# keillernogueira/dynamic-rs-segmentation

Measured on AMD Instinct MI355X. Metric: training patches/sec dilated_grsl_rate8 64x64x5, higher is better.
Workload: dtype f32; 1 GPU; dilated_grsl_rate8 (Dilated8Pooling) training step, single_fixed 64x64, 5-band synthetic 2048x2048 tile, global batch 128 (crop+augment+normalise, fwd, loss, bwd, momentum, confusion); global_batch=128, patch=64, bands=5, classes=6, parallelism=dp1, sync_bn=True, rccl_ranks_observed=1

## Files before the change

dynamic-rs-segmentation_amd/_lib.py:

```python
import ctypes as C
import os

_HERE = os.path.dirname(os.path.abspath(__file__))
LIB_PATH = os.path.join(_HERE, "libdrs_hip.so")
DEV_LIB_PATH = os.path.join(_HERE, "libdrs_hip_dev.so")

_p, _i, _f, _d = C.c_void_p, C.c_int, C.c_float, C.c_double
_sz, _u64 = C.c_size_t, C.c_ulonglong

SIGNATURES = {
    "drs_conv_mtile": (_i, [_i]),
    "drs_conv_forward": (_i, [_p, _i, _i, _i, _i, _i, _p, _p, _i, _i, _i, _i, _i, _p, _i, _i, _i, _p, _p]),
    "drs_conv_workspace_floats": (_sz, [_i]),
    "drs_conv_halo_skip": (_i, [_i, _i, _i, _i, _i, _i, _i]),
    "drs_conv_executed_ksteps": (_i, [_i, _i, _i, _i, _i, _i, _i, _p, _p]),
    "drs_conv_forward_ws": (_i, [_p, _i, _i, _i, _i, _i, _p, _p, _i, _i, _i, _i, _i, _p, _i, _i, _i, _p, _p, _sz, _p]),
    "drs_conv_wgrad_splits": (_i, [_i, _i, _i, _i, _i]),
    "drs_conv_wgrad": (_i, [_p, _i, _i, _i, _i, _i, _p, _i, _i, _i, _i, _i, _i, _i, _i, _i, _p, _p, _p]),
    "drs_filter_flip_transpose": (_i, [_p, _p, _i, _i, _i, _p]),
    "drs_filter_pad_cin": (_i, [_p, _p, _i, _i, _i, _i, _p]),
    "drs_split_conv_mtile": (_i, [_i]),
    "drs_split_terms": (_i, [_p, _sz, _i, _p, _p]),
    "drs_filter_split": (_i, [_p, _i, _i, _i, _i, _i, _p, _p, _p]),
    "drs_conv_forward_split": (_i, [_p, _i, _i, _i, _i, _i, _p, _p, _i, _i, _i, _i, _i, _p, _i, _i, _i, _p, _i, _p]),
# ... 74 lines not shown
    "drs_polygon_rings": (_i, [_p, _p, _i, _i, _i, _i, _p, _p, _p]),
    "drs_polygon_write": (_i, [_p, _i, _i, _i, _i, _i, _p, _p, _p, _p]),
    "drs_distance_scratch_bytes": (_sz, [_i, _i]),
    "drs_distance_transform": (_i, [_p, _p, _i, _i, _i, _i, _i, _p, _p, _sz, _p]),
    "drs_surface_scratch_bytes": (_sz, [_i, _i]),
    "drs_surface_histogram": (_i, [_p, _p, _i, _i, _i, _i, _p, _p, _sz, _p]),
    "drs_patch_boundary_weight": (_i, [_p, _p, _i, _i, _i, _d, _d, _p, _p, _p]),
    "drs_classifier_loss_pixel": (_i, [_p, _i, _i, _i, _i, _i, _i, _i, _p, _p, _p, _p, _p, _f, _p, _f, _p, _p, _p, _p, _i, _i, _p, _p,
                                       _p, _p, _p]),
    "drs_patch_dice_coeffs": (_i, [_p, _p, _p, _i, _i, _i, _d, _d, _d, _d, _p, _p, _p, _p]),
    "drs_classifier_loss_dice": (_i, [_p, _i, _i, _i, _i, _i, _i, _i, _p, _p, _p, _p, _p, _f, _p, _f, _p, _p, _p, _p, _p, _i, _i, _p,
                                      _p, _p, _p, _p]),
    "drs_dice_loss_add": (_i, [_p, _i, _p, _p]),
    "drs_patch_hard_weight": (_i, [_p, _p, _p, _p, _i, _i, _i, _d, _i, _p, _p, _p, _p]),
    "drs_lovasz_scratch_bytes": (_sz, [_i, _i, _i]),
    "drs_patch_lovasz_grad": (_i, [_p, _p, _p, _p, _i, _i, _i, _d, _p, _p, _p, _p, _p, _sz, _p]),
    "drs_classifier_loss_region": (_i, [_p, _i, _i, _i, _i, _i, _i, _i, _p, _p, _p, _p, _p, _f, _p, _f, _p, _p, _p, _p, _p, _i, _i, _p,
                                        _p, _p, _p, _p]),
    "drs_surface_loss_scratch_bytes": (_sz, [_i, _i, _i]),
    "drs_patch_surface_loss": (_i, [_p, _p, _p, _p, _i, _i, _i, _d, _d, _p, _i, _p, _p, _p, _p, _sz, _p]),
    "drs_net_create": (_i, [C.c_char_p, _i, _i, _f, _i, _i, _i, _f, C.POINTER(_p)]),
    "drs_net_destroy": (None, [_p]),
    "drs_net_num_buffers": (_i, [_p]),
    "drs_net_buffer_info": (_i, [_p, _i, C.c_char_p, _i, C.POINTER(_sz), C.POINTER(_i)]),
    "drs_net_bind": (_i, [_p, C.c_char_p, _p, _sz]),
    "drs_net_buffer": (_i, [_p, C.c_char_p, C.POINTER(_p), C.POINTER(_sz)]),
    "drs_net_layout": (_i, [_p, C.POINTER(_sz), C.POINTER(_sz), C.POINTER(_sz), C.POINTER(_i), C.POINTER(_i), C.POINTER(_i)]),
    "drs_net_layer_info": (_i, [_p, _i, C.c_char_p, _i, C.POINTER(_i), C.c_char_p, C.c_char_p, _i, C.POINTER(_i), C.POINTER(_i)]),
    "drs_net_info": (_i, [_p, C.c_char_p, _i, C.POINTER(_f), C.POINTER(_i), C.c_char_p, _i, C.POINTER(_i), C.POINTER(_i)]),
    "drs_net_receptive_field": (_i, [_p, C.POINTER(_i), C.POINTER(_i)]),
    "drs_net_receptive_field_gated": (_i, [_p, C.POINTER(_i), C.POINTER(_i)]),
    "drs_net_se_info": (_i, [_p, _i, C.c_char_p, _i, C.POINTER(_i), C.POINTER(_i), C.POINTER(_i)]),
    "drs_net_type_name": (_i, [_i, C.c_char_p, _i, C.POINTER(_i)]),
    "drs_net_num_variables": (_i, [_p]),
    "drs_net_variable_info": (_i, [_p, _i, C.c_char_p, _i, C.POINTER(_sz), C.POINTER(_sz), C.POINTER(_i), C.POINTER(_i)]),
    "drs_params_get": (_i, [_p, C.c_char_p, C.c_char_p, _p, _sz, _p]),
    "drs_params_set": (_i, [_p, C.c_char_p, C.c_char_p, _p, _sz, _p]),
    "drs_grad_buffer": (_i, [_p, C.POINTER(_p), C.POINTER(_sz)]),
    "drs_net_global_step": (C.c_longlong, [_p, C.c_longlong]),
    "drs_net_learning_rate": (_f, [_p, _f]),
    "drs_net_set_comm": (_i, [_p, _i, _i, _p, _p, _p]),
    "drs_rccl_bind_library": (_i, [C.c_char_p]),
    "drs_rccl_available": (_i, []),
    "drs_rccl_form": (_i, []),
    "drs_rccl_unique_id": (_i, [_p]),
    "drs_rccl_comm_create": (_i, [_i, _i, _p, C.POINTER(_p)]),
    "drs_rccl_comm_destroy": (_i, [_p]),
    "drs_rccl_all_reduce": (_i, [_p, _p, C.c_size_t, _i, _p]),
    "drs_net_set_rccl": (_i, [_p, _i, _i, _p, _p, _p]),
    "drs_train_step": (_i, [_p, _i, _i, _f, _i, _d, _p]),
    "drs_forward": (_i, [_p, _i, _i, _i, _i, _p]),
    "drs_apply_update": (_i, [_p, _f, _p]),
    "drs_forward_staged": (_i, [_p, _i, _i, _i, _p, _i, _i, _p]),
    "drs_net_se_gate_finish": (_i, [_p, _i, _d, _p]),
    "drs_net_set_two_streams": (_i, [_p, _i]),
    "drs_net_set_class_weights": (_i, [_p, _p, _i]),
    "drs_net_get_class_weights": (_i, [_p, _p, _i, C.POINTER(_i)]),
    "drs_net_set_focal_gamma": (_i, [_p, _f]),
    "drs_net_get_focal_gamma": (_i, [_p, C.POINTER(_f)]),
    "drs_net_set_boundary_weight": (_i, [_p, _d, _d, _i]),
    "drs_net_get_boundary_weight": (_i, [_p, C.POINTER(_d), C.POINTER(_d), C.POINTER(_i)]),
    "drs_net_set_dice": (_i, [_p, _d, _d, _d, _d]),
    "drs_net_get_dice": (_i, [_p, C.POINTER(_d), C.POINTER(_d), C.POINTER(_d), C.POINTER(_d)]),
    "drs_net_set_hard_mining": (_i, [_p, _d, _i]),
    "drs_net_get_hard_mining": (_i, [_p, C.POINTER(_d), C.POINTER(_i)]),
    "drs_net_set_lovasz": (_i, [_p, _d]),
    "drs_net_get_lovasz": (_i, [_p, C.POINTER(_d)]),
    "drs_net_set_surface_loss": (_i, [_p, _d, _d]),
    "drs_net_get_surface_loss": (_i, [_p, C.POINTER(_d), C.POINTER(_d)]),
    "drs_net_timing": (_i, [_p, _i]),
    "drs_net_num_timing_kinds": (_i, []),
    "drs_net_timing_summary": (_i, [_p, _i, C.c_char_p, _i, C.POINTER(_i), C.POINTER(_d), C.POINTER(_d)]),
}
ALLREDUCE_FN = C.CFUNCTYPE(_i, _p, _p, _sz, _i, _i, _p)
WAIT_FN = C.CFUNCTYPE(_i, _p, _i, _p)
WANT_LOGITS, WITH_LABELS, USE_ACC_MASK, USE_LOSS_MASK, NO_UPDATE = 1, 2, 4, 8, 16


DEV_SIGNATURES = {
    "drs_debug_skip_taps": (_i, [_i]), "drs_debug_conv_variant": (_i, [_i]), "drs_debug_conv_wide192": (_i, [_i]),
    "drs_debug_conv_splitk": (_i, [_i]), "drs_debug_conv_hybrid": (_i, [_i]), "drs_debug_conv_sk_order": (_i, [_i]), "drs_debug_conv_prio": (_i, [_i]),
    "drs_debug_conv_sk_geometry": (_i, [_i, _i, _i, _p]), "drs_debug_conv_trace": (_i, [_p]), "drs_debug_conv_lpt": (_i, [_i]), "drs_debug_conv_order": (_i, [_i] * 7 + [_p, _i]),
    "drs_debug_conv_image_tiles": (_i, [_i]), "drs_debug_conv_order_image": (_i, [_i] * 7 + [_p, _i]),
    "drs_debug_wgrad_variant": (_i, [_i]), "drs_debug_wgrad_seg": (_i, [_i]), "drs_debug_wgrad_balance": (_i, [_i]), "drs_debug_wgrad_target": (_i, [_i]),
    "drs_debug_wgrad_len": (_i, [_i]), "drs_debug_wgrad_minchunks": (_i, [_i]), "drs_debug_wgrad_prio": (_i, [_i]), "drs_debug_cls_variant": (_i, [_i]), "drs_debug_slide_blocks": (_i, [_i]), "drs_debug_slide_minrows": (_i, [_i]), "drs_debug_slide_rowpad": (_i, [_i]), "drs_debug_chain_mode": (_i, [_i]), "drs_debug_jitter": (_i, [C.c_ulonglong]), "drs_debug_wg_stream_prio": (_i, [_i]), "drs_debug_reductions_on_chain": (_i, [_i]), "drs_debug_wgrad_schedule": (_i, [_i, _i, _i]), "drs_debug_variant": (_i, [_i]),
    "drs_debug_wgrad_cut": (_i, [_i] * 7 + [_p, _i, _p, _p]),
}


class DrsError(RuntimeError):
    pass


_lib = None
_dev = None


def _open(path, signatures):
    if not os.path.isfile(path):
        raise DrsError("HIP library not built: %s is missing (run dynamic-rs-segmentation_amd/csrc/build.sh "
                       "or __graft_entry__.build()); there is no CPU fallback" % path)
    import torch
    lib = C.CDLL(path)
    for name, (res, args) in signatures.items():
        fn = getattr(lib, name)
        fn.restype = res
        fn.argtypes = args
    return lib


def load():
    global _lib
    if _lib is None:
        _lib = _open(LIB_PATH, SIGNATURES)
    return _lib


class _Dev(object):

    def __init__(self, lib):
        self.lib = lib

    def __getattr__(self, name):
        return getattr(self.lib, name)

    def load(self):
        return self.lib

    def call(self, name, *args):
        rc = getattr(self.lib, name)(*args)
        if rc != 0:
            raise DrsError("%s -> %s" % (name, _STATUS.get(rc, rc)))

    def query(self, name, *args):
        return getattr(self.lib, name)(*args)


def dev():
    global _dev
    if _dev is None:
        sig = dict(SIGNATURES)
        sig.update(DEV_SIGNATURES)
        _dev = _Dev(_open(DEV_LIB_PATH, sig))
    return _dev


_STATUS = {1: "DRS_ERR_ARG (rejected argument)", 2: "DRS_ERR_HIP (launch failed)"}


def call(name, *args):
    rc = getattr(load(), name)(*args)
    if rc != 0:
        raise DrsError("%s -> %s" % (name, _STATUS.get(rc, rc)))


def query(name, *args):
    return getattr(load(), name)(*args)
```

dynamic-rs-segmentation_amd/csrc/conv_mfma.hip:

```cpp
#include "drs_common.hpp"
#include <algorithm>
#include <cstdlib>
#include <map>
#include <mutex>
#include <numeric>
#include <tuple>
#include <vector>

namespace {

constexpr int BK = 32;
constexpr int LDA = BK + 4;

struct ConvArgs {
  const float* in; int S, P, ld_in, coff_in;
  int M;
  const float* w;
  const float* bias;
  float* out; int ld_out, coff_out;
  float* stats;
  int k, rate, pad, Cin, Cout;
  int accumulate;
  int skip_halo;
  float rcpS, rcpSS;
  float* sk_slab;
  int sk_W, sk_nks, sk_U;
  int sk_T, sk_tiles, sk_G, sk_order;
  int prio;
  int lpt_T, lpt_ta, lpt_tb, lpt_P;
  int img_g;
  const int* img_order;
#ifdef DRS_DEV
  unsigned long long* trace;
#endif
};

__device__ __forceinline__ void set_prio_by_progress(int done, int total, int& quarter, int mode = 1) {
  const int q = __builtin_amdgcn_readfirstlane((done * 4) / total);
  if (q == quarter) return;
  quarter = q;
  if (mode == 2) {
    if (q <= 0) __builtin_amdgcn_s_setprio(2);
    else if (q == 1) __builtin_amdgcn_s_setprio(1);
    else __builtin_amdgcn_s_setprio(0);
    return;
  }
  if (q <= 0) __builtin_amdgcn_s_setprio(3);
  else if (q == 1) __builtin_amdgcn_s_setprio(2);
  else if (q == 2) __builtin_amdgcn_s_setprio(1);
  else __builtin_amdgcn_s_setprio(0);
}

__host__ __device__ __forceinline__ int lpt_tile(int wg, int T, int ta, int tb, int P, int ntn) {
  const int per = P * T * ntn, nI = tb - ta, nE = T - nI;
  const int chunk = wg / per;
  int wl = wg - chunk * per, p, t;
  if (wl < P * nI * ntn) {
    p = wl / (nI * ntn);
    wl -= p * nI * ntn;
    t = ta + wl / ntn;
  } else {
    wl -= P * nI * ntn;
    p = wl / (nE * ntn);
    wl -= p * nE * ntn;
    const int e = wl / ntn;
    t = e < ta ? e : tb + (e - ta);
  }
  return ((chunk * P + p) * T + t) * ntn + wl % ntn;
}

__host__ __device__ __forceinline__ int sk_first_unit(int w, int U, int W) { return (int)((long long)w * U / W); }
__host__ __device__ __forceinline__ int sk_owner(int x, int U, int W) { return (int)((((long long)x + 1) * W - 1) / U); }

template <int BM, int BN, int WM, int WN, bool MAP = false>
__device__ __forceinline__ void conv_epilogue(const ConvArgs& a, f32x16 (&acc)[BM / WM / 32][BN / WN / 32], float* scratch, int m0, int n0,
                                              int pix0 = 0, int pcs = 30) {
  constexpr int WTM = BM / WM, WTN = BN / WN;
  constexpr int TM = WTM / 32, TN = WTN / 32;
  const int t = threadIdx.x;
  const int lane = t & 63, wave = t >> 6;
  const int li = lane & 31, h = lane >> 5;
  const int wm = wave / WN, wn = wave % WN;
  const int pcm = (1 << pcs) - 1, S2 = a.S * a.S;
  const int lane_rl = wm * WTM + 4 * h;
  const int lane_pix = MAP ? pix0 + (lane_rl >> pcs) * S2 + (lane_rl & pcm) : 0;
  float bv[TN];
#pragma unroll
  for (int ni = 0; ni < TN; ++ni) {
    const int col = n0 + wn * WTN + ni * 32 + li;
    bv[ni] = a.bias ? a.bias[col] : 0.f;
#pragma unroll
    for (int mi = 0; mi < TM; ++mi) {
#pragma unroll
      for (int r = 0; r < 16; ++r) {
        const int crl = mi * 32 + (r & 3) + 8 * (r >> 2);
        const int row = MAP ? lane_pix + __builtin_amdgcn_readfirstlane((crl >> pcs) * S2 + (crl & pcm)) : m0 + lane_rl + crl;
        if (row < a.M) {
          float v = acc[mi][ni][r] + bv[ni];
          float* dst = a.out + (size_t)row * a.ld_out + a.coff_out + col;
          if (a.accumulate) v += *dst;
          *dst = v;
        }
      }
    }
  }
  if (a.stats) {
    const int rem = a.M - m0;
    tile_column_stats<TN, WM, BN>(
        scratch, t, wm, h == 0, (float)(rem < BM ? rem : BM), [&](int ni) { return wn * WTN + ni * 32 + li; },
        [](float s) { return s + __shfl_xor(s, 32); },
        [&](int ni, auto f) {
#pragma unroll
          for (int mi = 0; mi < TM; ++mi)
#pragma unroll
            for (int r = 0; r < 16; ++r)
              if (m0 + wm * WTM + mi * 32 + (r & 3) + 8 * (r >> 2) + 4 * h < a.M) f(acc[mi][ni][r] + bv[ni]);
        },
        a.stats + ((size_t)(m0 / BM) * a.Cout + n0) * 2);
  }
}

template <int BM, int BN, int WM, int WN, bool PACK = false>
__global__ __launch_bounds__(256, (BM == 256 || BN == 128) ? 3 : 1) void conv_igemm_kernel(const ConvArgs a) {
  static_assert(WM * WN == 4, "4 waves");
  constexpr int LDB = BN + 4;
  constexpr int WTM = BM / WM, WTN = BN / WN;
  constexpr int TM = WTM / 32, TN = WTN / 32;
  constexpr int NA = BM / 32;
  constexpr int NB = BN / 32;
  constexpr int BROWS = 256 / (BN / 4);

  __shared__ __attribute__((aligned(16))) float lds[BM * LDA + BK * LDB];
  float* As = lds;
  float* Bs = lds + BM * LDA;

  const int t = threadIdx.x;
  const int lane = t & 63, wave = t >> 6;
  const int li = lane & 31, h = lane >> 5;
  const int wm = wave / WN, wn = wave % WN;

  const int ntn = a.Cout / BN;
  const int nblk = gridDim.x;
  const int tile = xcd_remap(blockIdx.x, nblk);
  const int m0 = (tile / ntn) * BM;
  const int n0 = (tile % ntn) * BN;

  const int Sp = a.S + 2 * a.P;
  uint32_t offA[NA];
#pragma unroll
  for (int i = 0; i < NA; ++i) {
    int p = m0 + (t >> 3) + 32 * i;
    p = p < a.M ? p : a.M - 1;
    offA[i] = (padded_pixel_off(p, a.S, a.P, a.ld_in, a.rcpS, a.rcpSS, -a.pad, -a.pad) + (uint32_t)(a.coff_in + (PACK ? 0 : (t & 7) * 4))) * 4u;
  }
  const int brow = t / (BN / 4), bcol = (t % (BN / 4)) * 4;
  uint32_t offB[NB];
#pragma unroll
  for (int i = 0; i < NB; ++i) offB[i] = (uint32_t)((brow + BROWS * i) * a.Cout + n0 + bcol) * 4u;

  f32x16 acc[TM][TN];
#pragma unroll
  for (int mi = 0; mi < TM; ++mi)
#pragma unroll
    for (int ni = 0; ni < TN; ++ni)
#pragma unroll
      for (int r = 0; r < 16; ++r) acc[mi][ni][r] = 0.f;

  const int cpt = a.Cin / BK;
  int u_lo, u_hi;
  live_tap_rows(m0, BM, a.M, a.S, a.k, a.rate, a.pad, a.rcpS, a.rcpSS, u_lo, u_hi);
  if (PACK || !a.skip_halo) { u_lo = 0; u_hi = a.k; }
  u_lo = __builtin_amdgcn_readfirstlane(u_lo);
  u_hi = __builtin_amdgcn_readfirstlane(u_hi);
  const int nks = PACK ? (a.k * a.k * a.Cin + BK - 1) / BK : (u_hi - u_lo) * a.k * cpt;
  const char* wlive = reinterpret_cast<const char*>(a.w + (size_t)u_lo * a.k * a.Cin * a.Cout);
  const char* inb = reinterpret_cast<const char*>(a.in);
  f32x4 ra[NA], rb[NB];
  int lu = u_lo, lv = 0, lc = 0;

  auto gload = [&](int ks) {
    if (PACK) {
      const int kidx = ks * BK + (t & 7) * 4;
      int tap = kidx / a.Cin;
      const int c = kidx - tap * a.Cin;
      tap = tap < a.k * a.k ? tap : a.k * a.k - 1;
      const int u = tap / a.k, v = tap - u * a.k;
      const uint32_t soff = (uint32_t)((u * a.rate * Sp + v * a.rate) * a.ld_in + c) * 4u;
#pragma unroll
      for (int i = 0; i < NA; ++i) ra[i] = *reinterpret_cast<const f32x4*>(inb + (offA[i] + soff));
    } else {
      const char* ab = inb + (size_t)(uint32_t)((lu * a.rate * Sp + lv * a.rate) * a.ld_in + lc * BK) * 4u;
#pragma unroll
      for (int i = 0; i < NA; ++i) { uint32_t o = offA[i]; asm volatile("" : "+v"(o)); ra[i] = *reinterpret_cast<const f32x4*>(ab + o); }
    }
    const char* wb = wlive + (size_t)(uint32_t)((PACK ? ks : ((lu - u_lo) * a.k + lv) * cpt + lc) * BK) * (uint32_t)a.Cout * 4u;
#pragma unroll
    for (int i = 0; i < NB; ++i) { uint32_t o = offB[i]; asm volatile("" : "+v"(o)); rb[i] = *reinterpret_cast<const f32x4*>(wb + o); }
    if (!PACK) { if (++lv == a.k) { lv = 0; if (++lu == u_hi) { lu = u_lo; ++lc; } } }
  };
  auto lstore = [&]() {
#pragma unroll
    for (int i = 0; i < NA; ++i) *reinterpret_cast<f32x4*>(&As[((t >> 3) + 32 * i) * LDA + (t & 7) * 4]) = ra[i];
// ... 993 lines not shown
  if (hipGetDevice(&dev) != hipSuccess || dev < 0 || dev >= 64) return 256;
  if (cached[dev] == 0) {
    hipDeviceProp_t p;
    cached[dev] = (hipGetDeviceProperties(&p, dev) == hipSuccess && p.multiProcessorCount >= 1) ? p.multiProcessorCount : 256;
  }
  return cached[dev];
}
inline int sk_max_w() { return 3 * cu_count(); }

struct SkGeom { int G, W, T; };
int g_conv_hybrid = 1;
SkGeom sk_geometry(int tiles, int nks, int bn, size_t ws_floats) {
  const SkGeom plain = {0, 0, 0};
  if (g_conv_splitk == 0 || tiles >= SK_MAX_TILES || nks < 2) return plain;
  const long long NCU = cu_count();
  long long cap = (long long)(ws_floats / (2ull * 128 * (size_t)bn));
  if (cap > sk_max_w()) cap = sk_max_w();
  if (cap < 1) return plain;
  const int MINU = 12;
  const int occ = 3;
  long long G, W, T = tiles;
  if (g_conv_splitk > 0) {
    G = W = g_conv_splitk;
  } else {
    const long long per = (tiles + NCU - 1) / NCU;
    if ((double)tiles >= 0.93 * (double)NCU * (double)per) return plain;
    const long long U = (long long)tiles * nks;
    long long per_cu = U / (NCU * MINU);
    per_cu = per_cu < 1 ? 1 : (per_cu > occ ? occ : per_cu);
    G = W = NCU * per_cu;
    if (U < NCU * MINU) G = W = U / MINU > 0 ? U / MINU : 1;
  }
  if (g_conv_hybrid && tiles > G) {
    T = tiles % G;
    if (T == 0) return plain;
    W = G;
  }
  if (W > T * nks) W = T * nks;
  if (W > G) W = G;
  if (W > cap) {
    if (g_conv_splitk <= 0) return plain;
    W = cap; if (G < W || T == tiles) G = W;
  }
  return SkGeom{(int)G, (int)W, (int)T};
}

void conv_lpt_setup(ConvArgs& a, int BM, int mt, int nt, int W) {
  a.lpt_T = 0; a.lpt_ta = a.lpt_tb = a.lpt_P = 0;
  if (W || !g_conv_lpt || drs_g_skip_halo_taps == 0) return;
  const int S2 = a.S * a.S, T = S2 % BM == 0 ? S2 / BM : 0, nblk = mt * nt;
  if (T < 2 || BM % a.S != 0 || nblk % 8 != 0 || (nblk / 8) % (T * nt) != 0) return;
  const int rows = BM / a.S;
  auto full = [&](int t) {
    const int y0 = t * rows, y1 = y0 + rows - 1;
    const int lo = a.pad - y1 > 0 ? (a.pad - y1 + a.rate - 1) / a.rate : 0;
    int hi = (a.S - 1 - y0 + a.pad) / a.rate + 1;
    hi = hi < a.k ? hi : a.k;
    return lo == 0 && hi == a.k;
  };
  int ta = 0, tb = T;
  while (ta < T && !full(ta)) ++ta;
  while (tb > ta && !full(tb - 1)) --tb;
  bool ok = ta < tb;
  for (int t = ta; ok && t < tb; ++t) ok = full(t);
  if (ok && (ta > 0 || tb < T)) { a.lpt_T = T; a.lpt_ta = ta; a.lpt_tb = tb; a.lpt_P = nblk / 8 / (T * nt); a.skip_halo = 1; }
}

int g_conv_image_tiles = -1;

int conv_image_tiles_rule(int k, int rate, int cin, int cout, int B, int S) {
  if (B != 128 || S != 64) return 0;
  struct Row { int k, rate, cin, cout; };
  static const Row gains[] = {{4, 3, 64, 128},
                              {4, 4, 128, 128},
                              {3, 5, 128, 192}, {3, 5, 192, 128},
                              {3, 6, 192, 192},
                              {3, 7, 192, 256}, {3, 7, 256, 192},
                              {3, 8, 256, 256}};
  for (const Row& r : gains)
    if (r.k == k && r.rate == rate && r.cin == cin && r.cout == cout) return 7;
  return 0;
}

int conv_image_tiles_g(int B, int S, int k, int rate, int cin, int cout) {
  const int g = g_conv_image_tiles < 0 ? conv_image_tiles_rule(k, rate, cin, cout, B, S) : g_conv_image_tiles;
  if (g < 4 || g > 7 || k < 2 || cin < BK || cin % BK || g_conv_variant == 0) return 0;
  if (B % (1 << g) || S % (128 >> g)) return 0;
  return g;
}

inline int image_tile_taps(int mt, int S, int k, int rate, int pad, int g) {
  int y, x0, ul, uh, vl, vh;
  image_tile_pos(mt, S, g, y, x0);
  live_taps_image_tile(y, x0, 128 >> g, S, k, rate, pad, ul, uh, vl, vh);
  return (uh - ul) * (vh - vl);
}

std::vector<int> conv_image_order(int B, int S, int k, int rate, int pad, int g) {
  const int mt = B * S * S / 128;
  std::vector<int> taps(mt), sorted(mt), order(mt);
  for (int i = 0; i < mt; ++i) taps[i] = image_tile_taps(i, S, k, rate, pad, g);
  std::iota(sorted.begin(), sorted.end(), 0);
  std::stable_sort(sorted.begin(), sorted.end(), [&](int x, int y) { return taps[x] > taps[y]; });
  if (mt % 8) return sorted;
  const int per = mt / 8;
  for (int c = 0; c < 8; ++c)
    for (int j = 0; j < per; ++j) order[c * per + j] = sorted[j * 8 + c];
  return order;
}

const int* conv_image_order_device(int B, int S, int k, int rate, int pad, int g) {
  static std::mutex mu;
  static std::map<std::tuple<int, int, int, int, int, int, int>, const int*> cache;
  int dev = 0;
  if (hipGetDevice(&dev) != hipSuccess) return nullptr;
  std::lock_guard<std::mutex> lock(mu);
  const auto key = std::make_tuple(dev, B, S, k, rate, pad, g);
  const auto it = cache.find(key);
  if (it != cache.end()) return it->second;
  const std::vector<int> order = conv_image_order(B, S, k, rate, pad, g);
  int* d = nullptr;
  if (hipMalloc((void**)&d, order.size() * sizeof(int)) != hipSuccess) return nullptr;
  if (hipMemcpy(d, order.data(), order.size() * sizeof(int), hipMemcpyHostToDevice) != hipSuccess) { (void)hipFree(d); return nullptr; }
  cache[key] = d;
  return d;
}

template <int BM, int BN, int WM, int WN>
int launch_conv_dma(ConvArgs& a, float* ws, size_t ws_floats, hipStream_t st) {
  const int mt = (a.M + BM - 1) / BM, nt = a.Cout / BN;
  const int nks = a.k * a.k * (a.Cin / BK);
  const SkGeom g = ws && (reinterpret_cast<uintptr_t>(ws) & 15) == 0 ? sk_geometry(mt * nt, nks, BN, ws_floats) : SkGeom{0, 0, 0};
  const int W = g.W;
  a.sk_W = W; a.sk_nks = nks; a.sk_U = g.T * nks; a.sk_slab = ws;
  a.sk_T = g.T; a.sk_tiles = mt * nt; a.sk_G = g.G; a.sk_order = g_conv_sk_order;
  a.prio = g_conv_prio >= 0 ? g_conv_prio : (g.G && (long long)mt * nt * nks >= 20LL * g.G ? 1 : 0);
  if (g_conv_prio < 0 && drs_chain_level(drs_tl_chain, drs_g_chain_mode) >= 1) a.prio = 3;
  conv_lpt_setup(a, BM, mt, nt, g.G);
  if (!g.G && !a.stats) {
    const int B = a.M / (a.S * a.S);
    a.img_g = conv_image_tiles_g(B, a.S, a.k, a.rate, a.Cin, a.Cout);
    if (a.img_g) {
      a.img_order = conv_image_order_device(B, a.S, a.k, a.rate, a.pad, a.img_g);
      if (!a.img_order) return DRS_ERR_HIP;
      a.lpt_T = 0;
      a.skip_halo = drs_g_skip_halo_taps != 0;
    }
  }
  if (g.G) DRS_LAUNCH((conv_dma_kernel<BM, BN, WM, WN, true>), dim3(g.G), dim3(256), 0, st, a);
  else DRS_LAUNCH((conv_dma_kernel<BM, BN, WM, WN, false>), dim3(mt * nt), dim3(256), 0, st, a);
  int rc = DRS_LAUNCH_CHECK();
  if (rc || !g.G) return rc;
  if (a.sk_U % W == 0 && (a.sk_U / W) % nks == 0) return rc;
  DRS_LAUNCH((conv_sk_fixup_kernel<BM, BN, WM, WN>), dim3(g.T), dim3(256), 0, st, a);
  return DRS_LAUNCH_CHECK();
}

template <int BM, int BN, int WM, int WN>
int launch_conv(ConvArgs& a, float* ws, size_t ws_floats, hipStream_t st) {
  const int mt = (a.M + BM - 1) / BM, nt = a.Cout / BN;
  if (a.Cin < BK) DRS_LAUNCH((conv_igemm_kernel<BM, BN, WM, WN, true>), dim3(mt * nt), dim3(256), 0, st, a);
  else if constexpr (BM == 128) {
    const bool dma = g_conv_variant != 0;
    if (dma) return launch_conv_dma<BM, BN, WM, WN>(a, ws, ws_floats, st);
    DRS_LAUNCH((conv_igemm_kernel<BM, BN, WM, WN>), dim3(mt * nt), dim3(256), 0, st, a);
  } else DRS_LAUNCH((conv_igemm_kernel<BM, BN, WM, WN>), dim3(mt * nt), dim3(256), 0, st, a);
  return DRS_LAUNCH_CHECK();
}

int g_wgrad_variant = -1;

inline bool wgrad_affine(const WgradArgs& a) { return (a.S & 31) == 0; }
int g_wgrad_seg = 1;
inline bool wgrad_segments(const WgradArgs& a) {
  const long long Sxp = a.S + 2 * a.Px, Sgp = a.S + 2 * a.Pg, B = a.M / ((long long)a.S * a.S);
  const long long xb = (B * Sxp * Sxp + 64) * a.ld_x * 4, gb = (B * Sgp * Sgp + 64) * a.ld_g * 4;
  return g_wgrad_seg && a.S >= 32 && !wgrad_affine(a) && xb < (1LL << 32) && gb < (1LL << 32);
}

template <int TR, int TO>
int launch_wgrad(const WgradArgs& a, int nwg, hipStream_t st) {
  constexpr int NT = 64 * (TR >= 64 ? 2 : 1) * (TO >= 64 ? 2 : 1);
  const bool dma = g_wgrad_variant < 0 ? (TO == 128 || (TO == 64 && (wgrad_affine(a) || (wgrad_segments(a) && a.M < (1 << 18))))) : g_wgrad_variant == 1;
  if (!dma && wgrad_affine(a)) DRS_LAUNCH((wgrad_kernel<TR, TO, true>), dim3(nwg), dim3(NT), 0, st, a);
  else if (!dma) DRS_LAUNCH((wgrad_kernel<TR, TO, false>), dim3(nwg), dim3(NT), 0, st, a);
  else if (wgrad_affine(a)) DRS_LAUNCH((wgrad_dma_kernel<TR, TO, 1>), dim3(nwg), dim3(NT), 0, st, a);
  else if (wgrad_segments(a)) DRS_LAUNCH((wgrad_dma_kernel<TR, TO, 2>), dim3(nwg), dim3(NT), 0, st, a);
  else DRS_LAUNCH((wgrad_dma_kernel<TR, TO, 0>), dim3(nwg), dim3(NT), 0, st, a);
  return DRS_LAUNCH_CHECK();
}

template <int TR, int TO>
int launch_wgrad_dma_only(const WgradArgs& a, int nwg, hipStream_t st) {
  if (wgrad_affine(a)) DRS_LAUNCH((wgrad_dma_kernel<TR, TO, 1>), dim3(nwg), dim3(256), 0, st, a);
  else if (wgrad_segments(a)) DRS_LAUNCH((wgrad_dma_kernel<TR, TO, 2>), dim3(nwg), dim3(256), 0, st, a);
  else DRS_LAUNCH((wgrad_dma_kernel<TR, TO, 0>), dim3(nwg), dim3(256), 0, st, a);
  return DRS_LAUNCH_CHECK();
}

}

__attribute__((visibility("hidden"))) int drs_step_prep(const StepPrepArgs& a, hipStream_t stream) {
  if (a.n < 0 || a.n > STEP_PREP_MAX) return DRS_ERR_ARG;
  DRS_LAUNCH(step_prep_kernel, dim3(512, a.n + 2), dim3(256), 0, stream, a);
  return DRS_LAUNCH_CHECK();
}


int drs_g_skip_halo_taps = 1;
thread_local int drs_tl_chain = 0;
int drs_g_chain_mode = -1;

namespace {

int g_wgrad_target = 2048;

int pick_tile(int c) { return c % 128 == 0 ? 128 : (c % 64 == 0 ? 64 : 32); }
int g_conv_wide192 = 1;
int pick_conv_tile(int c, int cin) { return (g_conv_wide192 && c % 192 == 0 && c % 128 != 0 && cin % 32 == 0 && g_conv_variant != 0) ? 192 : pick_tile(c); }

int pick_wgrad_rows(int rows) {
  const int n128 = (rows + 127) / 128;
  if ((double)rows / (n128 * 128.0) >= 0.85) return 128;
  if (rows % 64 == 0) return 64;
  return rows % 32 == 0 && rows < 128 ? 32 : 128;
}

int pick_wgrad_cols(int tr, int cout) { return (tr == 128 && cout % 192 == 0 && cout % 128 != 0 && g_wgrad_variant != 0) ? 192 : pick_tile(cout); }

int g_wgrad_balance = 1;
int g_wgrad_len = 0;
inline int wgrad_len(int nchunks) { return g_wgrad_len ? g_wgrad_len : (nchunks >= (1 << 14) ? 192 : 96); }
int g_wgrad_minchunks = 8;

// ... 119 lines not shown
  a.x = nullptr; a.g = nullptr; a.slab = nullptr; a.Px = a.Pg = a.ld_x = a.ld_g = a.coff_x = a.coff_g = 0;
  a.S = S; a.M = (int)M;
  a.k = k; a.rate = rate; a.pad = pad_before; a.Cin = cin; a.Cout = cout;
  tr = pick_wgrad_rows(k * k * cin); to = pick_wgrad_cols(tr, cout);
  a.ntr = (k * k * cin + tr - 1) / tr; a.nto = cout / to;
  nsplit = wgrad_uniform_splits(B, S, k, cin, cout);
  const int nchunks = (int)((M + 31) / 32);
  a.chunks_per_split = (nchunks + nsplit - 1) / nsplit;
  a.rcpS = 1.0f / (float)S; a.rcpSS = 1.0f / (float)(S * S);
  a.prio = g_wgrad_prio >= 0 ? g_wgrad_prio : (M >= (1LL << 18) ? 1 : 0);
#ifdef DRS_DEV
  a.trace = g_conv_trace;
#endif
  nwg = nsplit * a.ntr * a.nto;
  a.plan.nclass = 0;
  a.live_cut = 0;
  if (g_wgrad_balance && wgrad_live_plan(B, S, k, rate, pad_before, cin, cout, tr, to, wgrad_bound_splits(B, S, k, cin, cout), a.plan, nwg)) {
    a.live_cut = 1;
    a.skip_halo = drs_g_skip_halo_taps != 0;
  } else {
    a.skip_halo = drs_skip_halo_taps_wgrad(M);
    a.live_cut = a.skip_halo;
  }
  return DRS_OK;
}

int conv_plain_image_g(int B, int S, int k, int rate, int cin, int cout) {
  if (cin < 32 || cin % 32) return 0;
  const int bn = pick_conv_tile(cout, cin);
  if (bn < 64) return 0;
  const int mt = (int)(((long long)B * S * S + 127) / 128), nt = cout / bn;
  if (sk_geometry(mt * nt, k * k * (cin / 32), bn, 2ull * (size_t)sk_max_w() * 128 * (size_t)bn).G) return 0;
  return conv_image_tiles_g(B, S, k, rate, cin, cout);
}

}

extern "C" {

#ifdef DRS_DEV
int drs_debug_skip_taps(int v) { const int old = drs_g_skip_halo_taps; if (v >= 0) drs_g_skip_halo_taps = v; return old; }

int drs_debug_wgrad_target(int v) { const int old = g_wgrad_target; if (v > 0) g_wgrad_target = v; return old; }

int drs_debug_wgrad_balance(int v) { const int old = g_wgrad_balance; if (v >= 0) g_wgrad_balance = v; return old; }

int drs_debug_wgrad_len(int v) { const int old = g_wgrad_len; if (v >= 0) g_wgrad_len = v; return old; }

int drs_debug_wgrad_minchunks(int v) { const int old = g_wgrad_minchunks; if (v > 0) g_wgrad_minchunks = v; return old; }

int drs_debug_wgrad_prio(int v) { const int old = g_wgrad_prio; if (v >= -1) g_wgrad_prio = v; return old; }

int drs_debug_conv_wide192(int v) { const int old = g_conv_wide192; if (v >= 0) g_conv_wide192 = v; return old; }

int drs_debug_conv_variant(int v) { const int old = g_conv_variant; if (v >= -1) g_conv_variant = v; return old; }

size_t drs_conv_workspace_floats(int cout);
int drs_debug_conv_lpt(int v) { const int old = g_conv_lpt; if (v >= 0) g_conv_lpt = v; return old; }
int drs_debug_conv_order(int B, int S, int k, int rate, int pad_before, int cin, int cout, int* out, int cap) {
  const long long M = (long long)B * S * S;
  if (M <= 0 || M >= (1 << 24) || cout % 32 || k < 1 || rate < 1) return -1;
  ConvArgs a;
  a.S = S; a.M = (int)M; a.k = k; a.rate = rate; a.pad = pad_before; a.Cin = cin; a.Cout = cout;
  a.skip_halo = drs_skip_halo_taps_fwd(M, cout);
  const int bn = pick_conv_tile(cout, cin);
  if (bn < 64) return 0;
  const int mt = (int)((M + 127) / 128), nt = cout / bn;
  const int W = cin >= 32 ? sk_geometry(mt * nt, k * k * (cin / 32), bn, drs_conv_workspace_floats(cout)).G : 0;
  conv_lpt_setup(a, 128, mt, nt, W);
  if (!a.lpt_T) return 0;
  for (int w = 0; w < mt * nt && w < cap; ++w) out[w] = lpt_tile(w, a.lpt_T, a.lpt_ta, a.lpt_tb, a.lpt_P, nt);
  return mt * nt;
}
int drs_debug_conv_image_tiles(int g) { const int old = g_conv_image_tiles; if (g >= -1) g_conv_image_tiles = g; return old; }
int drs_debug_conv_order_image(int B, int S, int k, int rate, int pad_before, int cin, int cout, int* out, int cap) {
  const long long M = (long long)B * S * S;
  if (M <= 0 || M >= (1 << 24) || cout % 32 || k < 1 || rate < 1) return -1;
  const int g = conv_plain_image_g(B, S, k, rate, cin, cout);
  if (!g) return 0;
  const int mt = (int)(M / 128), nt = cout / pick_conv_tile(cout, cin);
  const std::vector<int> order = conv_image_order(B, S, k, rate, pad_before, g);
  for (int w = 0; w < mt * nt && w < cap; ++w) out[w] = order[w / nt] * nt + w % nt;
  return mt * nt;
}
int drs_debug_conv_trace(void* dev_buffer) { g_conv_trace = (unsigned long long*)dev_buffer; return 0; }

int drs_debug_conv_splitk(int v) { const int old = g_conv_splitk; if (v >= -1) g_conv_splitk = v; return old; }
int drs_debug_conv_hybrid(int v) { const int old = g_conv_hybrid; if (v >= 0) g_conv_hybrid = v; return old; }
int drs_debug_conv_sk_order(int v) { const int old = g_conv_sk_order; if (v >= 0) g_conv_sk_order = v; return old; }
int drs_debug_chain_mode(int v) { const int old = drs_g_chain_mode; if (v >= -1) drs_g_chain_mode = v; return old; }
int drs_debug_conv_prio(int v) { const int old = g_conv_prio; if (v >= -1) g_conv_prio = v; return old; }
int drs_debug_conv_sk_geometry(int tiles, int nks, int bn, int* out3) {
  const SkGeom g = sk_geometry(tiles, nks, bn, 2ull * (size_t)sk_max_w() * 128 * (size_t)bn);
  if (out3) { out3[0] = g.G; out3[1] = g.W; out3[2] = g.T; }
  return g.G;
}

int drs_debug_wgrad_variant(int v) { const int old = g_wgrad_variant; if (v >= -1) g_wgrad_variant = v; return old; }
int drs_debug_wgrad_seg(int v) { const int old = g_wgrad_seg; if (v >= 0) g_wgrad_seg = v; return old; }

#endif

int drs_conv_mtile(int cout) { return pick_tile(cout) >= 64 ? 128 : 256; }

size_t drs_conv_workspace_floats(int cout) {
  const int bn = pick_conv_tile(cout, 32);
  return bn >= 64 ? 2ull * (size_t)sk_max_w() * 128 * (size_t)bn : 0;
}

int drs_conv_halo_skip(int B, int S, int k, int rate, int pad_before, int cin, int cout) {
  const long long M = (long long)B * S * S;
  if (M <= 0 || M >= (1 << 24) || cout % 32 || cin < 32 || cin % 32 || k < 1 || rate < 1) return 0;
  ConvArgs a;
  a.S = S; a.M = (int)M; a.k = k; a.rate = rate; a.pad = pad_before; a.Cin = cin; a.Cout = cout;
  a.skip_halo = drs_skip_halo_taps_fwd(M, cout);
  const int bn = pick_conv_tile(cout, cin);
  if (bn < 64) return a.skip_halo;
  const int mt = (int)((M + 127) / 128), nt = cout / bn;
  const int W = sk_geometry(mt * nt, k * k * (cin / 32), bn, drs_conv_workspace_floats(cout)).G;
  if (W) return 0;
  conv_lpt_setup(a, 128, mt, nt, 0);
  return a.skip_halo;
}

int drs_conv_executed_ksteps(int B, int S, int k, int rate, int pad_before, int cin, int cout, long long* executed, long long* total) {
  const long long M = (long long)B * S * S;
  if (B < 1 || S < 1 || M >= (1 << 24) || cout < 32 || cout % 32 || cin < 1 || k < 1 || rate < 1 || !executed || !total) return DRS_ERR_ARG;
  const int bn = pick_conv_tile(cout, cin), bm = bn >= 64 ? 128 : 256;
  const int mt = (int)((M + bm - 1) / bm), nt = cout / bn;
  const long long cpt = cin < 32 ? 1 : cin / 32;
  *total = *executed = cin < 32 ? (long long)mt * nt * ((k * k * cin + 31) / 32) : (long long)mt * nt * k * k * cpt;
  if (cin < 32 || cin % 32) return DRS_OK;
  const int g = conv_plain_image_g(B, S, k, rate, cin, cout);
  long long taps = 0;
  if (g) {
    if (drs_g_skip_halo_taps == 0) return DRS_OK;
    for (int i = 0; i < mt; ++i) taps += image_tile_taps(i, S, k, rate, pad_before, g);
  } else {
    if (!drs_conv_halo_skip(B, S, k, rate, pad_before, cin, cout)) return DRS_OK;
    for (int i = 0; i < mt; ++i) {
      const int p0 = i * bm, p1 = (int)(p0 + bm < M ? p0 + bm : M) - 1;
      int y0 = (p0 % (S * S)) / S, y1 = (p1 % (S * S)) / S;
      if (p0 / (S * S) != p1 / (S * S)) { y0 = 0; y1 = S - 1; }
      int lo = pad_before - y1 > 0 ? (pad_before - y1 + rate - 1) / rate : 0, hi = (S - 1 - y0 + pad_before) / rate + 1;
      hi = hi < k ? hi : k;
      if (lo >= hi) { lo = 0; hi = k; }
      taps += (hi - lo) * k;
    }
  }
  *executed = taps * nt * cpt;
  return DRS_OK;
}

int drs_conv_forward_ws(const float* in, int B, int S, int P, int ld_in, int coff_in, const float* w, const float* bias,
                        int k, int rate, int pad_before, int cin, int cout, float* out, int ld_out, int coff_out,
                        int accumulate, float* stats_partial, float* workspace, size_t workspace_floats, void* stream) {
  if (!in || !w || !out || (cin % 32 && cin != 8 && cin != 16) || cout % 32 || k < 1 || rate < 1 || P < pad_before) return DRS_ERR_ARG;
  if (B < 1 || S < 1 || cin < 8 || cout < 32 || pad_before < 0 || !drs_prod_below(1LL << 31, {k, k, cin, cout})) return DRS_ERR_ARG;
  if (coff_in < 0 || ld_in < coff_in + cin || coff_out < 0 || ld_out < coff_out + cout) return DRS_ERR_ARG;
  if (cin < 32 && (ld_in % 4 || coff_in % 4)) return DRS_ERR_ARG;
  if (accumulate && stats_partial) return DRS_ERR_ARG;
  if (P < (long long)(k - 1) * rate - pad_before) return DRS_ERR_ARG;
  const long long M = (long long)B * S * S;
  if (M <= 0 || M >= (1 << 24)) return DRS_ERR_ARG;
  if ((long long)B * (S + 2 * P) * (S + 2 * P) * ld_in >= (1LL << 30)) return DRS_ERR_ARG;
  ConvArgs a;
// ... 100 lines not shown
```

dynamic-rs-segmentation_amd/csrc/drs_common.hpp:

```cpp
#pragma once
#include <hip/hip_runtime.h>
#include <stdint.h>
#include <initializer_list>

#define DRS_OK 0
#define DRS_ERR_ARG 1
#define DRS_ERR_HIP 2

typedef float f32x4 __attribute__((ext_vector_type(4)));
typedef float f32x16 __attribute__((ext_vector_type(16)));

struct ActView {
  float* base;
  int S;
  int P;
  int ld;
  int coff;
  uint16_t* terms;
  int nt;
};

__device__ __forceinline__ void view_store4(const ActView& v, size_t e, f32x4 x) {
  if (v.base) *reinterpret_cast<f32x4*>(v.base + e) = x;
  if (v.terms) {
// ... 15 lines not shown
  q = (int)((float)n * rcp);
  r = n - q * d;
  if (r < 0) { q -= 1; r += d; }
  else if (r >= d) { q += 1; r -= d; }
}

__device__ __forceinline__ uint32_t padded_pixel_off(int p, int S, int P, int ld, float rcpS, float rcpSS, int dy, int dx) {
  int b, rem, y, x;
  divmod24(p, S * S, rcpSS, b, rem);
  divmod24(rem, S, rcpS, y, x);
  const int Sp = S + 2 * P;
  return (uint32_t)(((b * Sp + y + P + dy) * Sp + (x + P + dx))) * (uint32_t)ld;
}

constexpr int STEP_PREP_MAX = 24;
struct StepPrepArgs {
  const float* w[STEP_PREP_MAX];
  float* wt[STEP_PREP_MAX];
  int k[STEP_PREP_MAX], cin[STEP_PREP_MAX], cout[STEP_PREP_MAX];
  int n;
  unsigned int* z0; int nz0;
  float* z1; int nz1;
};

__device__ __forceinline__ void live_tap_rows(int m0, int BM, int M, int S, int k, int rate, int pad, float rcpS, float rcpSS,
                                              int& lo, int& hi) {
  const int p1 = (m0 + BM - 1 < M ? m0 + BM : M) - 1;
  int b0, r0, b1, r1, y0, y1, x;
  divmod24(m0, S * S, rcpSS, b0, r0);
  divmod24(p1, S * S, rcpSS, b1, r1);
  divmod24(r0, S, rcpS, y0, x);
  divmod24(r1, S, rcpS, y1, x);
  if (b0 != b1) { y0 = 0; y1 = S - 1; }
  const int a = pad - y1;
  lo = a > 0 ? (a + rate - 1) / rate : 0;
  const int bnum = S - 1 - y0 + pad;
  hi = bnum / rate + 1;
  hi = hi < k ? hi : k;
  if (lo >= hi) { lo = 0; hi = k; }
}

__host__ __device__ __forceinline__ void live_taps_image_tile(int y, int x0, int Pc, int S, int k, int rate, int pad,
                                                              int& u_lo, int& u_hi, int& v_lo, int& v_hi) {
  const int au = pad - y, av = pad - (x0 + Pc - 1);
  u_lo = au > 0 ? (au + rate - 1) / rate : 0;
  v_lo = av > 0 ? (av + rate - 1) / rate : 0;
  u_hi = (S - 1 - y + pad) / rate + 1;
  v_hi = (S - 1 - x0 + pad) / rate + 1;
  u_hi = u_hi < k ? u_hi : k;
  v_hi = v_hi < k ? v_hi : k;
  if (u_lo >= u_hi || v_lo >= v_hi) { u_lo = v_lo = 0; u_hi = v_hi = k; }
}
__host__ __device__ __forceinline__ int image_tile_pos(int mt, int S, int g, int& y, int& x0) {
  const int Pc = 128 >> g, npc = S / Pc;
  const int t2 = mt / npc;
  x0 = (mt - t2 * npc) * Pc;
  const int grp = t2 / S;
  y = t2 - grp * S;
  return grp;
}

__host__ __device__ __forceinline__ void live_pixel_range(int row_first, int row_last, int Cin, int k, int rate, int pad, int S, int enable,
                                                          int& lo, int& hi) {
  const int dy_min = (row_first / Cin / k) * rate - pad, dy_max = (row_last / Cin / k) * rate - pad;
  int ylo = -dy_max > 0 ? -dy_max : 0;
  int yhi = S - dy_min < S ? S - dy_min : S;
  if (!enable || ylo >= yhi) { ylo = 0; yhi = S; }
  lo = ylo * S;
  hi = yhi * S;
}

__device__ __forceinline__ int next_live_chunk(int c, int S2, float rcpSS, int lo, int hi) {
  const int p = 32 * (c + 1);
  int b, r;
  divmod24(p, S2, rcpSS, b, r);
  if (r + 31 >= lo && r < hi) return c + 1;
  if (r + 31 >= S2 + lo) return c + 1;
  return ((r < lo ? b : b + 1) * S2 + lo) >> 5;
}

template <int NSLOT, int WM, int BN, class Col, class LaneSum, class Each>
__device__ __forceinline__ void tile_column_stats(float* red, int t, int wm, bool writer, float n_tile, Col col, LaneSum lanesum,
                                                  Each each, float* dst) {
  float* red2 = red + WM * BN;
#pragma unroll
  for (int ni = 0; ni < NSLOT; ++ni) {
    float s = 0.f;
    each(ni, [&](float v) { s += v; });
    s = lanesum(s);
    if (writer) red[wm * BN + col(ni)] = s;
  }
  __syncthreads();
  const float rn = 1.0f / n_tile;
#pragma unroll
  for (int ni = 0; ni < NSLOT; ++ni) {
    float tot = 0.f;
#pragma unroll
    for (int w = 0; w < WM; ++w) tot += red[w * BN + col(ni)];
    const float mean = tot * rn;
    float q = 0.f;
    each(ni, [&](float v) { const float d = v - mean; q += d * d; });
    q = lanesum(q);
    if (writer) red2[wm * BN + col(ni)] = q;
  }
  __syncthreads();
  if (t >= 0 && t < BN && dst) {
    float u1 = 0.f, u2 = 0.f;
#pragma unroll
    for (int w = 0; w < WM; ++w) { u1 += red[w * BN + t]; u2 += red2[w * BN + t]; }
    dst[2 * t] = u1;
    dst[2 * t + 1] = u2;
  }
}

inline int drs_chain_level(int asked, int mode) { return asked == 0 ? 0 : (mode < 0 ? asked : mode); }
extern thread_local int drs_tl_chain;
extern int drs_g_chain_mode;

extern int drs_g_skip_halo_taps;
static inline int drs_skip_halo_taps_fwd(long long M, int cout) {
  if (drs_g_skip_halo_taps != 1) return drs_g_skip_halo_taps == 2;
  const long long wgs = ((M + 127) / 128) * ((cout + 127) / 128);
  return wgs >= 4096;
}
static inline int drs_skip_halo_taps_wgrad(long long M) {
  if (drs_g_skip_halo_taps != 1) return drs_g_skip_halo_taps == 2;
  return M >= (1LL << 19);
}

__device__ __forceinline__ int xcd_remap(int bid, int nblk) {
  const int xcd = bid & 7, q = nblk >> 3, r = nblk & 7;
  const int start = xcd < r ? xcd * (q + 1) : r * (q + 1) + (xcd - r) * q;
  return start + (bid >> 3);
}

static inline bool drs_prod_below(long long lim, std::initializer_list<long long> f) {
  long long p = 1;
  for (long long v : f) {
    if (v < 1 || v >= lim) return false;
    p *= v;
    if (p >= lim) return false;
  }
  return true;
}
static inline bool drs_slice_ok(int ld, int coff, int C, int align) {
  return C >= 1 && coff >= 0 && (long long)coff + C <= ld && ld % align == 0 && coff % align == 0;
}
static inline bool drs_rows_ok(int B, int S, int P) {
  return B >= 1 && S >= 1 && P >= 0 && (long long)B * ((long long)S + 2LL * P) <= 65535;
}

static inline int drs_check(hipError_t e) { return e == hipSuccess ? DRS_OK : DRS_ERR_HIP; }
#define DRS_LAUNCH_CHECK() drs_check(hipGetLastError())
#define DRS_LAUNCH(...) do { (void)hipGetLastError(); hipLaunchKernelGGL(__VA_ARGS__); } while (0)
```

include/drs_dev.h:

```cpp
#ifndef DRS_DEV_H_
#define DRS_DEV_H_
#ifdef __cplusplus
extern "C" {
#endif

int drs_debug_skip_taps(int v);
int drs_debug_conv_variant(int v);
int drs_debug_conv_wide192(int v);
int drs_debug_conv_lpt(int v);
int drs_debug_conv_order(int B, int S, int k, int rate, int pad_before, int cin, int cout, int* out, int cap);
int drs_debug_conv_image_tiles(int g);
int drs_debug_conv_order_image(int B, int S, int k, int rate, int pad_before, int cin, int cout, int* out, int cap);
int drs_debug_conv_trace(void* dev_buffer);
int drs_debug_conv_splitk(int v);
int drs_debug_conv_hybrid(int v);
int drs_debug_conv_sk_order(int v);
int drs_debug_conv_prio(int v);
int drs_debug_conv_sk_geometry(int tiles, int nks, int bn, int* out3);
int drs_debug_wgrad_variant(int v);
int drs_debug_wgrad_seg(int v);
int drs_debug_wgrad_balance(int v);
int drs_debug_wgrad_target(int v);
int drs_debug_wgrad_len(int v);
int drs_debug_wgrad_minchunks(int v);
int drs_debug_wgrad_prio(int v);
int drs_debug_slide_blocks(int v);
int drs_debug_slide_minrows(int v);
int drs_debug_jitter(unsigned long long seed);
int drs_debug_wg_stream_prio(int arm);
int drs_debug_reductions_on_chain(int on);
int drs_debug_wgrad_schedule(int layer_slabs, int streams, int defer);
int drs_debug_chain_mode(int v);
int drs_debug_slide_rowpad(int v);
int drs_debug_cls_variant(int v);
int drs_debug_variant(int v);
int drs_debug_wgrad_cut(int B, int S, int k, int rate, int pad_before, int cin, int cout, int* out, int cap, int* out_tile_splits,
                        int* out_tile_rows);

#ifdef __cplusplus
}
#endif
#endif
```

Before: 2694 patches/s.

## Enable image-tile ordering for stats convs via separate per-tile stats kernel

Convolutions that also produce batch-norm column statistics could not use the image-tile launch order before, because stats were computed in the epilogue. They now run the image-ordered conv kernel without stats, then a separate kernel rereads the output and computes per-tile column sums and variances. A shape-keyed rule turns this on for four dilated layer shapes at batch 128, patch 64. The gain in cache locality from image-tile order is paid for with an extra kernel launch and a full reread of the output. The stats reduction also gets fp contract(fast).

```diff
diff --git a/dynamic-rs-segmentation_amd/_lib.py b/dynamic-rs-segmentation_amd/_lib.py
--- a/dynamic-rs-segmentation_amd/_lib.py
+++ b/dynamic-rs-segmentation_amd/_lib.py
@@ -180,6 +180,7 @@
     "drs_debug_conv_splitk": (_i, [_i]), "drs_debug_conv_hybrid": (_i, [_i]), "drs_debug_conv_sk_order": (_i, [_i]), "drs_debug_conv_prio": (_i, [_i]),
     "drs_debug_conv_sk_geometry": (_i, [_i, _i, _i, _p]), "drs_debug_conv_trace": (_i, [_p]), "drs_debug_conv_lpt": (_i, [_i]), "drs_debug_conv_order": (_i, [_i] * 7 + [_p, _i]),
     "drs_debug_conv_image_tiles": (_i, [_i]), "drs_debug_conv_order_image": (_i, [_i] * 7 + [_p, _i]),
+    "drs_debug_conv_tile_stats": (_i, [_p, _i, _i, _i, _i, _i, _p, _i, _p]),
     "drs_debug_wgrad_variant": (_i, [_i]), "drs_debug_wgrad_seg": (_i, [_i]), "drs_debug_wgrad_balance": (_i, [_i]), "drs_debug_wgrad_target": (_i, [_i]),
     "drs_debug_wgrad_len": (_i, [_i]), "drs_debug_wgrad_minchunks": (_i, [_i]), "drs_debug_wgrad_prio": (_i, [_i]), "drs_debug_cls_variant": (_i, [_i]), "drs_debug_slide_blocks": (_i, [_i]), "drs_debug_slide_minrows": (_i, [_i]), "drs_debug_slide_rowpad": (_i, [_i]), "drs_debug_chain_mode": (_i, [_i]), "drs_debug_jitter": (_i, [C.c_ulonglong]), "drs_debug_wg_stream_prio": (_i, [_i]), "drs_debug_reductions_on_chain": (_i, [_i]), "drs_debug_wgrad_schedule": (_i, [_i, _i, _i]), "drs_debug_variant": (_i, [_i]),
     "drs_debug_wgrad_cut": (_i, [_i] * 7 + [_p, _i, _p, _p]),
diff --git a/dynamic-rs-segmentation_amd/csrc/conv_mfma.hip b/dynamic-rs-segmentation_amd/csrc/conv_mfma.hip
--- a/dynamic-rs-segmentation_amd/csrc/conv_mfma.hip
+++ b/dynamic-rs-segmentation_amd/csrc/conv_mfma.hip
@@ -72,6 +72,25 @@
 __host__ __device__ __forceinline__ int sk_first_unit(int w, int U, int W) { return (int)((long long)w * U / W); }
 __host__ __device__ __forceinline__ int sk_owner(int x, int U, int W) { return (int)((((long long)x + 1) * W - 1) / U); }
 
+template <int BM, int BN, int WM, int WN, class Val>
+__device__ __forceinline__ void conv_tile_stats(float* stats, int M, int Cout, float* scratch, int m0, int n0, int t, int wm, int wn, int li,
+                                                int h, Val val) {
+  constexpr int WTM = BM / WM, WTN = BN / WN;
+  constexpr int TM = WTM / 32, TN = WTN / 32;
+  const int rem = M - m0;
+  tile_column_stats<TN, WM, BN>(
+      scratch, t, wm, h == 0, (float)(rem < BM ? rem : BM), [&](int ni) { return wn * WTN + ni * 32 + li; },
+      [](float s) { return s + __shfl_xor(s, 32); },
+      [&](int ni, auto f) {
+#pragma unroll
+        for (int mi = 0; mi < TM; ++mi)
+#pragma unroll
+          for (int r = 0; r < 16; ++r)
+            if (m0 + wm * WTM + mi * 32 + (r & 3) + 8 * (r >> 2) + 4 * h < M) f(val(mi, ni, r));
+      },
+      stats + ((size_t)(m0 / BM) * Cout + n0) * 2);
+}
+
 template <int BM, int BN, int WM, int WN, bool MAP = false>
 __device__ __forceinline__ void conv_epilogue(const ConvArgs& a, f32x16 (&acc)[BM / WM / 32][BN / WN / 32], float* scratch, int m0, int n0,
                                               int pix0 = 0, int pcs = 30) {
@@ -105,19 +124,38 @@
     }
   }
   if (a.stats) {
-    const int rem = a.M - m0;
-    tile_column_stats<TN, WM, BN>(
-        scratch, t, wm, h == 0, (float)(rem < BM ? rem : BM), [&](int ni) { return wn * WTN + ni * 32 + li; },
-        [](float s) { return s + __shfl_xor(s, 32); },
-        [&](int ni, auto f) {
-#pragma unroll
-          for (int mi = 0; mi < TM; ++mi)
-#pragma unroll
-            for (int r = 0; r < 16; ++r)
-              if (m0 + wm * WTM + mi * 32 + (r & 3) + 8 * (r >> 2) + 4 * h < a.M) f(acc[mi][ni][r] + bv[ni]);
-        },
-        a.stats + ((size_t)(m0 / BM) * a.Cout + n0) * 2);
-  }
+    conv_tile_stats<BM, BN, WM, WN>(a.stats, a.M, a.Cout, scratch, m0, n0, t, wm, wn, li, h,
+                                    [&](int mi, int ni, int r) { return acc[mi][ni][r] + bv[ni]; });
+  }
+}
+
+template <int BM, int BN, int WM, int WN>
+__global__ __launch_bounds__(256) void conv_tile_stats_kernel(const float* __restrict__ out, int ld_out, int coff_out, int M, int Cout,
+                                                              float* __restrict__ stats, int desc) {
+  constexpr int WTM = BM / WM, WTN = BN / WN;
+  constexpr int TM = WTM / 32, TN = WTN / 32;
+  __shared__ float red[2 * WM * BN];
+  const int t = threadIdx.x;
+  const int lane = t & 63, wave = t >> 6;
+  const int li = lane & 31, h = lane >> 5;
+  const int wm = wave / WN, wn = wave % WN;
+  const int ntn = Cout / BN;
+  int mtile = blockIdx.x / ntn;
+  const int n0 = (blockIdx.x - mtile * ntn) * BN;
+  if (desc) mtile = (int)(gridDim.x / ntn) - 1 - mtile;
+  const int m0 = mtile * BM;
+  const float* src = out + (size_t)(m0 + wm * WTM + 4 * h) * ld_out + coff_out + n0 + wn * WTN + li;
+  f32x16 v[TM][TN];
+#pragma unroll
+  for (int mi = 0; mi < TM; ++mi)
+#pragma unroll
+    for (int ni = 0; ni < TN; ++ni)
+#pragma unroll
+      for (int r = 0; r < 16; ++r) {
+        const int crl = mi * 32 + (r & 3) + 8 * (r >> 2);
+        v[mi][ni][r] = m0 + wm * WTM + 4 * h + crl < M ? src[(size_t)crl * ld_out + ni * 32] : 0.f;
+      }
+  conv_tile_stats<BM, BN, WM, WN>(stats, M, Cout, red, m0, n0, t, wm, wn, li, h, [&](int mi, int ni, int r) { return v[mi][ni][r]; });
 }
 
 template <int BM, int BN, int WM, int WN, bool PACK = false>
@@ -1277,8 +1315,21 @@
   return 0;
 }
 
-int conv_image_tiles_g(int B, int S, int k, int rate, int cin, int cout) {
-  const int g = g_conv_image_tiles < 0 ? conv_image_tiles_rule(k, rate, cin, cout, B, S) : g_conv_image_tiles;
+int conv_image_tiles_stats_rule(int k, int rate, int cin, int cout, int B, int S) {
+  if (B != 128 || S != 64) return 0;
+  struct Row { int k, rate, cin, cout; };
+  static const Row gains[] = {{4, 4, 128, 128},
+                              {3, 6, 192, 192},
+                              {3, 7, 192, 256},
+                              {3, 8, 256, 256}};
+  for (const Row& r : gains)
+    if (r.k == k && r.rate == rate && r.cin == cin && r.cout == cout) return 7;
+  return 0;
+}
+
+int conv_image_tiles_g(int B, int S, int k, int rate, int cin, int cout, bool stats = false) {
+  const int g = g_conv_image_tiles >= 0 ? g_conv_image_tiles
+                                        : (stats ? conv_image_tiles_stats_rule(k, rate, cin, cout, B, S) : conv_image_tiles_rule(k, rate, cin, cout, B, S));
   if (g < 4 || g > 7 || k < 2 || cin < BK || cin % BK || g_conv_variant == 0) return 0;
   if (B % (1 << g) || S % (128 >> g)) return 0;
   return g;
@@ -1332,19 +1383,28 @@
   a.prio = g_conv_prio >= 0 ? g_conv_prio : (g.G && (long long)mt * nt * nks >= 20LL * g.G ? 1 : 0);
   if (g_conv_prio < 0 && drs_chain_level(drs_tl_chain, drs_g_chain_mode) >= 1) a.prio = 3;
   conv_lpt_setup(a, BM, mt, nt, g.G);
-  if (!g.G && !a.stats) {
+  float* stats_from_out = nullptr;
+  if (!g.G && !(a.stats && a.accumulate)) {
     const int B = a.M / (a.S * a.S);
-    a.img_g = conv_image_tiles_g(B, a.S, a.k, a.rate, a.Cin, a.Cout);
+    a.img_g = conv_image_tiles_g(B, a.S, a.k, a.rate, a.Cin, a.Cout, a.stats != nullptr);
     if (a.img_g) {
       a.img_order = conv_image_order_device(B, a.S, a.k, a.rate, a.pad, a.img_g);
       if (!a.img_order) return DRS_ERR_HIP;
       a.lpt_T = 0;
       a.skip_halo = drs_g_skip_halo_taps != 0;
+      stats_from_out = a.stats;
+      a.stats = nullptr;
     }
   }
   if (g.G) DRS_LAUNCH((conv_dma_kernel<BM, BN, WM, WN, true>), dim3(g.G), dim3(256), 0, st, a);
   else DRS_LAUNCH((conv_dma_kernel<BM, BN, WM, WN, false>), dim3(mt * nt), dim3(256), 0, st, a);
   int rc = DRS_LAUNCH_CHECK();
+  if (stats_from_out) {
+    a.stats = stats_from_out;
+    if (rc) return rc;
+    DRS_LAUNCH((conv_tile_stats_kernel<BM, BN, WM, WN>), dim3(mt * nt), dim3(256), 0, st, a.out, a.ld_out, a.coff_out, a.M, a.Cout, a.stats, 0);
+    return DRS_LAUNCH_CHECK();
+  }
   if (rc || !g.G) return rc;
   if (a.sk_U % W == 0 && (a.sk_U / W) % nks == 0) return rc;
   DRS_LAUNCH((conv_sk_fixup_kernel<BM, BN, WM, WN>), dim3(g.T), dim3(256), 0, st, a);
@@ -1630,6 +1690,20 @@
   const std::vector<int> order = conv_image_order(B, S, k, rate, pad_before, g);
   for (int w = 0; w < mt * nt && w < cap; ++w) out[w] = order[w / nt] * nt + w % nt;
   return mt * nt;
+}
+int drs_debug_conv_tile_stats(const float* out, int B, int S, int cout, int ld_out, int coff_out, float* stats, int descending, void* stream) {
+  const long long M = (long long)B * S * S;
+  if (!out || !stats || B < 1 || S < 1 || M >= (1 << 24) || cout < 64 || cout % 64 || !drs_slice_ok(ld_out, coff_out, cout, 1)) return DRS_ERR_ARG;
+  if (M * ld_out >= (1LL << 31)) return DRS_ERR_ARG;
+  const int bn = pick_conv_tile(cout, 32), mt = (int)((M + 127) / 128), nt = cout / bn, desc = descending != 0;
+  hipStream_t st = (hipStream_t)stream;
+  switch (bn) {
+    case 192: DRS_LAUNCH((conv_tile_stats_kernel<128, 192, 2, 2>), dim3(mt * nt), dim3(256), 0, st, out, ld_out, coff_out, (int)M, cout, stats, desc); break;
+    case 128: DRS_LAUNCH((conv_tile_stats_kernel<128, 128, 2, 2>), dim3(mt * nt), dim3(256), 0, st, out, ld_out, coff_out, (int)M, cout, stats, desc); break;
+    case 64:  DRS_LAUNCH((conv_tile_stats_kernel<128, 64, 2, 2>), dim3(mt * nt), dim3(256), 0, st, out, ld_out, coff_out, (int)M, cout, stats, desc); break;
+    default:  return DRS_ERR_ARG;
+  }
+  return DRS_LAUNCH_CHECK();
 }
 int drs_debug_conv_trace(void* dev_buffer) { g_conv_trace = (unsigned long long*)dev_buffer; return 0; }
 
diff --git a/dynamic-rs-segmentation_amd/csrc/drs_common.hpp b/dynamic-rs-segmentation_amd/csrc/drs_common.hpp
--- a/dynamic-rs-segmentation_amd/csrc/drs_common.hpp
+++ b/dynamic-rs-segmentation_amd/csrc/drs_common.hpp
@@ -121,6 +121,7 @@
 template <int NSLOT, int WM, int BN, class Col, class LaneSum, class Each>
 __device__ __forceinline__ void tile_column_stats(float* red, int t, int wm, bool writer, float n_tile, Col col, LaneSum lanesum,
                                                   Each each, float* dst) {
+#pragma clang fp contract(fast)
   float* red2 = red + WM * BN;
 #pragma unroll
   for (int ni = 0; ni < NSLOT; ++ni) {
diff --git a/include/drs_dev.h b/include/drs_dev.h
--- a/include/drs_dev.h
+++ b/include/drs_dev.h
@@ -11,6 +11,7 @@
 int drs_debug_conv_order(int B, int S, int k, int rate, int pad_before, int cin, int cout, int* out, int cap);
 int drs_debug_conv_image_tiles(int g);
 int drs_debug_conv_order_image(int B, int S, int k, int rate, int pad_before, int cin, int cout, int* out, int cap);
+int drs_debug_conv_tile_stats(const float* out, int B, int S, int cout, int ld_out, int coff_out, float* stats, int descending, void* stream);
 int drs_debug_conv_trace(void* dev_buffer);
 int drs_debug_conv_splitk(int v);
 int drs_debug_conv_hybrid(int v);
```

Result: no change. 2715 patches/s (median of 6 runs) (+0.8%).
